# salemmohammed/Distributed-TensorFlow-Guide

Hardware: AMD Instinct MI355X
Metric: images/sec (whole node) ResNet-50 sync DP at 1/2/4/8 MI355X; scaling efficiency (higher is better)
Workload: dtype bf16; 1 GPU; model=ResNet-50, global_batch=1024, per_gpu_batch=1024, image_size=224, optimizer=momentum-sgd (fused), parallelism=dp1, allreduce=rccl bf16, 8 MB buckets, overlapped, step_launch=eager

## Files before the change

### csrc/bindings/ops.cc

```cpp
#include <torch/extension.h>
#include <c10/core/DeviceGuard.h>
#include <c10/hip/HIPStream.h>

#include "dtg/kernels.h"

namespace {

using at::Tensor;
using dtg::bf16_t;

hipStream_t cur_stream() { return c10::hip::getCurrentHIPStream().stream(); }

at::Tensor zeros_f32(long long n, const at::Tensor& like) {
  c10::DeviceGuard dg(like.device());
  at::Tensor t = at::empty({n}, like.options().dtype(at::kFloat));
  dtg::fill_zero(t.data_ptr(), n * 4, cur_stream());
  return t;
}

#define CHECK_CUDA(x) TORCH_CHECK((x).is_cuda(), #x " must be a GPU tensor")
#define CHECK_CONTIG(x) TORCH_CHECK((x).is_contiguous(), #x " must be contiguous")
#define CHECK_DT(x, dt) TORCH_CHECK((x).scalar_type() == (dt), #x " must be " #dt)
#define CHECK_IN(x) \
  CHECK_CUDA(x);    \
// ... 987 lines not shown
  CHECK_IN(x);
  CHECK_DT(x, at::kBFloat16);
  TORCH_CHECK(x.dim() == 2, "x must be [M, C]");
  const long long M = x.size(0);
  const int C = (int)x.size(1);
  TORCH_CHECK(C % 8 == 0, "C must be a multiple of 8");
  check_partials({&part}, C);
  check_per_channel({&gamma, &beta, &rmean, &rvar}, C);
  const bool has_res = res.has_value() && res->defined();
  if (has_res) {
    CHECK_IN(*res);
    CHECK_DT(*res, at::kBFloat16);
    TORCH_CHECK(res->sizes() == x.sizes(), "residual shape mismatch");
  }
  c10::DeviceGuard dg(x.device());
  auto y = at::empty_like(x);
  auto fopt = x.options().dtype(at::kFloat);
  auto smean = at::empty({C}, fopt), sinv = at::empty({C}, fopt), ws = at::empty({2LL * C}, fopt);
  dtg::bn_fwd_from_part(cbfp(x), has_res ? cbfp(*res) : nullptr, bfp(y), gamma.data_ptr<float>(),
                        beta.data_ptr<float>(), rmean.data_ptr<float>(), rvar.data_ptr<float>(),
                        smean.data_ptr<float>(), sinv.data_ptr<float>(), part.data_ptr<float>(), ws.data_ptr<float>(),
                        M, C, (float)momentum, (float)eps, relu, cur_stream(), bits_ptr(bits, M, C));
  return {y, smean, sinv};
}

std::tuple<Tensor, Tensor, Tensor, Tensor, Tensor> bn_fwd2_part(Tensor x, Tensor part, Tensor gamma, Tensor beta,
                                                                Tensor rmean, Tensor rvar, Tensor r, Tensor part2,
                                                                Tensor gamma2, Tensor beta2, Tensor rmean2,
                                                                Tensor rvar2, double momentum, double eps,
                                                                c10::optional<Tensor> bits) {
  CHECK_IN(x);
  CHECK_IN(r);
  CHECK_DT(x, at::kBFloat16);
  CHECK_DT(r, at::kBFloat16);
  TORCH_CHECK(x.dim() == 2 && r.sizes() == x.sizes(), "x/r must be [M, C]");
  const long long M = x.size(0);
  const int C = (int)x.size(1);
  TORCH_CHECK(C % 8 == 0, "C must be a multiple of 8");
  check_partials({&part, &part2}, C);
  check_per_channel({&gamma, &beta, &rmean, &rvar, &gamma2, &beta2, &rmean2, &rvar2}, C);
  c10::DeviceGuard dg(x.device());
  auto y = at::empty_like(x);
  auto fopt = x.options().dtype(at::kFloat);
  auto m1 = at::empty({C}, fopt), i1 = at::empty({C}, fopt), m2 = at::empty({C}, fopt), i2 = at::empty({C}, fopt);
  auto ws = at::empty({4LL * C}, fopt);
  dtg::bn_fwd2_from_part(cbfp(x), cbfp(r), bfp(y), part.data_ptr<float>(), part2.data_ptr<float>(),
// ... 256 lines not shown
  m.def("bn_dx_wgrad_ok", [](int64_t M, int64_t C, int64_t CI) { return dtg::bn_dx_wgrad_ok(M, (int)C, (int)CI); });
  m.def("bn_dx_dgrad_ok", [](int64_t M, int64_t C, int64_t CI) { return dtg::bn_dx_dgrad_ok(M, (int)C, (int)CI); });
  m.def("bn_dx_dgrad_full_ok",
        [](int64_t M, int64_t C, int64_t CI) { return dtg::bn_dx_dgrad_full_ok(M, (int)C, (int)CI); });
  m.def("bn_dx_wgrad_slabs",
        [](int64_t C, int64_t CI, int64_t w2, bool dg) { return dtg::bn_dx_wgrad_slabs((int)C, (int)CI, (int)w2, dg); },
        pybind11::arg("C"), pybind11::arg("CI"), pybind11::arg("w2") = 0, pybind11::arg("dg") = false);
  m.def("conv_fwd_bn", &conv_fwd_bn, pybind11::arg("x"), pybind11::arg("w"), pybind11::arg("stride"),
        pybind11::arg("pad"), pybind11::arg("pooled") = false);
  m.def("conv_dgrad_bn", &conv_dgrad_bn, pybind11::arg("dy"), pybind11::arg("w"), pybind11::arg("H"),
        pybind11::arg("W"), pybind11::arg("stride"), pybind11::arg("pad"), pybind11::arg("x"), pybind11::arg("mean"),
        pybind11::arg("invstd"), pybind11::arg("gamma"), pybind11::arg("beta"), pybind11::arg("pooled") = false,
        pybind11::arg("bits") = pybind11::none());
  m.def("bn_fwd2_part", &bn_fwd2_part, pybind11::arg("x"), pybind11::arg("part"), pybind11::arg("gamma"),
        pybind11::arg("beta"), pybind11::arg("rmean"), pybind11::arg("rvar"), pybind11::arg("r"), pybind11::arg("part2"),
        pybind11::arg("gamma2"), pybind11::arg("beta2"), pybind11::arg("rmean2"), pybind11::arg("rvar2"),
        pybind11::arg("momentum"), pybind11::arg("eps"), pybind11::arg("bits") = pybind11::none());
  m.def("conv_fwd_c8", &conv_fwd_c8, pybind11::arg("x"), pybind11::arg("w"), pybind11::arg("R"), pybind11::arg("S"),
        pybind11::arg("stride"), pybind11::arg("pad"), pybind11::arg("with_stats") = false,
        pybind11::arg("stride_w") = 0);
  m.def("bn_fwd_part", &bn_fwd_part, pybind11::arg("x"), pybind11::arg("part"), pybind11::arg("res"),
        pybind11::arg("gamma"), pybind11::arg("beta"), pybind11::arg("rmean"), pybind11::arg("rvar"),
        pybind11::arg("momentum"), pybind11::arg("eps"), pybind11::arg("relu"), pybind11::arg("bits") = pybind11::none());
  m.def("bn_bwd_part", &bn_bwd_part, pybind11::arg("dp"), pybind11::arg("x"), pybind11::arg("part"),
        pybind11::arg("gamma"), pybind11::arg("smean"), pybind11::arg("sinv"), pybind11::arg("want_dres"),
        pybind11::arg("dgamma_acc") = pybind11::none(), pybind11::arg("dbeta_acc") = pybind11::none(),
        pybind11::arg("wact") = pybind11::none(), pybind11::arg("wgrad") = pybind11::none(),
        pybind11::arg("dgw") = pybind11::none(), pybind11::arg("dgy") = pybind11::none(),
        pybind11::arg("dgmean") = pybind11::none(), pybind11::arg("dginv") = pybind11::none(),
        pybind11::arg("dgbits") = pybind11::none(), pybind11::arg("dgpart") = pybind11::none(),
        pybind11::arg("dgfull") = false);
  m.doc() = "dtg gfx950 HIP kernels";
  {
    namespace py = pybind11;
    m.def("sgd_apply", &sgd_apply, py::arg("w"), py::arg("mirror"), py::arg("g"), py::arg("hyper"), py::arg("wd"),
          py::arg("gscale"), py::arg("zero_grad"), py::arg("clip") = py::none());
    m.def("momentum_apply", &momentum_apply, py::arg("w"), py::arg("mirror"), py::arg("g"), py::arg("mom"),
          py::arg("hyper"), py::arg("mu"), py::arg("wd"), py::arg("nesterov"), py::arg("gscale"), py::arg("zero_grad"),
          py::arg("clip") = py::none());
    m.def("adagrad_apply", &adagrad_apply, py::arg("w"), py::arg("mirror"), py::arg("g"), py::arg("acc"),
          py::arg("hyper"), py::arg("eps"), py::arg("gscale"), py::arg("zero_grad"), py::arg("clip") = py::none());
    m.def("adam_apply", &adam_apply, py::arg("w"), py::arg("mirror"), py::arg("g"), py::arg("m"), py::arg("v"),
          py::arg("hyper"), py::arg("b1"), py::arg("b2"), py::arg("eps"), py::arg("wd"), py::arg("gscale"),
          py::arg("zero_grad"), py::arg("clip") = py::none());
  }
  m.attr("LW_CHUNK") = (int)dtg::kLwChunk;
// ... 28 lines not shown
      sbytes = scratch->numel() * scratch->element_size();
      dev_t = &*scratch;
    }
    if (bucket.has_value() && bucket->defined()) {
      CHECK_IN(*bucket);
      TORCH_CHECK(bucket->scalar_type() == at::kFloat || bucket->scalar_type() == at::kBFloat16, "bucket fp32/bf16");
      n = bucket->numel();
      bf = bucket->scalar_type() == at::kBFloat16;
      dev_t = &*bucket;
    }
    TORCH_CHECK(!(mode & 2) || sbytes > 0, "traffic mode needs scratch");
    TORCH_CHECK(!(mode & 4) || n > 0 || !(bucket.has_value() && bucket->defined()), "data mode needs the bucket");
    c10::optional<c10::DeviceGuard> dg;
    if (dev_t) dg.emplace(dev_t->device());
    return dtg::comm_emu(seconds, (int)wgs, (int)mode, sbytes ? scratch->data_ptr() : nullptr, sbytes, base,
                         traffic_bytes, n ? bucket->data_ptr() : nullptr, n, bf, (float)factor, cur_stream());
  }, pybind11::arg("seconds"), pybind11::arg("wgs") = 32, pybind11::arg("mode") = 0,
        pybind11::arg("scratch") = pybind11::none(), pybind11::arg("base") = 0, pybind11::arg("traffic_bytes") = 0,
        pybind11::arg("bucket") = pybind11::none(), pybind11::arg("factor") = 1.0);
  m.def("stem_stream_set", [](int64_t on) { dtg::stem_stream_set((int)on); });
  m.def("gemm_expand_k256_set", [](int64_t on) { dtg::gemm_expand_k256_set((int)on); });
  m.def("stem_pool_rows_set", [](int64_t on) { dtg::stem_pool_rows_set((int)on); });
  m.def("gemm_expand_s2_set", [](int64_t on) { dtg::gemm_expand_s2_set((int)on); });
  m.def("conv_halo_fwd_set", [](int64_t on) { dtg::conv3x3_halo_fwd_set((int)on); });
  m.def("conv_halo_dgrad_set", [](int64_t on) { dtg::conv3x3_halo_dgrad_set((int)on); });
  m.def("conv_halo_wgrad_set", [](int64_t on) { dtg::conv3x3_halo_wgrad_set((int)on); });
  m.def("conv_lin_wgrad_set", [](int64_t on) { dtg::conv3x3_lin_wgrad_set((int)on); });
  m.def("hyper_tick", [](Tensor hyper) {
    check_hyper(hyper);
    c10::DeviceGuard dg(hyper.device());
    dtg::hyper_tick(hyper.data_ptr<float>(), cur_stream());
  });
  m.def("stem_pack_weights", [](Tensor w) {
    CHECK_CUDA(w);
    CHECK_DT(w, at::kBFloat16);
    TORCH_CHECK(w.dim() == 4 && w.is_contiguous(at::MemoryFormat::ChannelsLast) && w.size(1) <= 4,
                "w: channels_last [K, C<=4, R, S]");
    const int K = w.size(0), C = w.size(1), R = w.size(2), S = w.size(3), S2 = (S + 1) / 2;
    const int KP = (R * S2 * 8 + 63) / 64 * 64;
    c10::DeviceGuard dg(w.device());
    auto wp = at::empty({K, KP}, w.options().memory_format(at::MemoryFormat::Contiguous));
    dtg::stem_pack_weights(cbfp(w), bfp(wp), K, C, R, S, S2, KP, cur_stream());
    return wp;
  });
  m.def("stem_dw_add", [](Tensor src, Tensor grad, bool pair) {
    CHECK_IN(src);
// ... 63 lines not shown
```

### csrc/include/dtg/kernels.h

```cpp
#pragma once
#include <hip/hip_runtime.h>
#include <stdint.h>

namespace dtg {
typedef unsigned short bf16_t;

void sgd_apply(float* w, bf16_t* mirror, void* grad, int grad_bf16, long long n, const float* hyper, float wd,
               float gscale, int zero_grad, hipStream_t st, const float* clip = nullptr);
void momentum_apply(float* w, bf16_t* mirror, void* grad, int grad_bf16, float* mom, long long n,
                    const float* hyper, float mu, float wd, int nesterov, float gscale, int zero_grad,
                    hipStream_t st, const float* clip = nullptr);
void adagrad_apply(float* w, bf16_t* mirror, void* grad, int grad_bf16, float* acc, long long n,
                   const float* hyper, float eps, float gscale, int zero_grad, hipStream_t st,
                   const float* clip = nullptr);
void adam_apply(float* w, bf16_t* mirror, void* grad, int grad_bf16, float* m, float* v, long long n,
                const float* hyper, float b1, float b2, float eps, float wd, float gscale, int zero_grad,
                hipStream_t st, const float* clip = nullptr);
void axpby(float* acc, const void* g, int g_bf16, long long n, float alpha, float beta, hipStream_t st);
void f32_to_bf16(const float* x, bf16_t* y, long long n, hipStream_t st);
void hyper_tick(float* hyper, hipStream_t st);
struct GradSrcs {
  const void* p[8] = {nullptr, nullptr, nullptr, nullptr, nullptr, nullptr, nullptr, nullptr};
};
void sgd_sum_apply(float* w, bf16_t* mirror, const float* acc, const GradSrcs& src, int k, int src_bf16, long long n,
// ... 235 lines not shown
int conv_supported(int C, int K, int R, int S, int stride, int pad, int which);
int conv3x3_halo_bn_ok(int C, int K, int H, int W);
bool conv3x3_halo_bn_fwd(const bf16_t* x, const bf16_t* w, bf16_t* y, int N, int H, int W, float* part, hipStream_t st);
void conv3x3_halo_fwd_set(int on);
bool conv3x3_halo_bn_dgrad(const bf16_t* dy, const bf16_t* w, bf16_t* dp, int N, int H, int W, const BnEpi& bn,
                           hipStream_t st);
void conv3x3_halo_dgrad_set(int on);
int conv3x3_halo_wgrad_split(int N, int H, int W, int C, int K, int R, int S, int stride, int pad, int stride_w);
void conv3x3_halo_wgrad(const bf16_t* dy, const bf16_t* x, float* ws, int grid, int N, int H, hipStream_t st);
void conv3x3_halo_wgrad_set(int on);
int conv3x3_lin_wgrad_split(int N, int H, int W, int C, int K, int R, int S, int stride, int pad, int stride_w);
void conv3x3_lin_wgrad(const bf16_t* dy, const bf16_t* x, float* ws, int split, int N, int H, int W, int C, int K,
                       hipStream_t st);
void conv3x3_lin_wgrad_set(int on);
void conv_fwd(const bf16_t* x, const bf16_t* w, bf16_t* y, int N, int H, int W, int C, int K, int R, int S,
              int stride, int pad, hipStream_t st, const BnEpi& bn = BnEpi());
int conv_dgrad(const bf16_t* dy, const bf16_t* w, bf16_t* dx, int N, int H, int W, int C, int K, int R, int S,
               int stride, int pad, float beta, hipStream_t st, const BnEpi& bn = BnEpi(),
               const bf16_t* wT = nullptr, int zero_rest = 1);
void stem_stream_set(int on);
void stem_pool_rows_set(int on);
void gemm_expand_k256_set(int on);
void gemm_expand_s2_set(int on);
bool conv1x1_s2_expand_bn(const bf16_t* x, int Nb, int H, int W, int Cin, const bf16_t* w, bf16_t* y, int Kout,
                          float* part, hipStream_t st);
void conv_fwd_c8(const bf16_t* x, const bf16_t* w, bf16_t* y, int N, int H, int W, int K, int R, int S, int stride,
                 int pad, hipStream_t st, const BnEpi& bn = BnEpi(), int stride_w = 0);
void conv_set_stages(int which, int stages);
int conv_wgrad_split(int N, int H, int W, int C, int K, int R, int S, int stride, int pad, int stride_w = 0,
                     int target_wgs = 0);
void conv_wgrad(const bf16_t* dy, const bf16_t* x, void* dw, int dw_bf16, float beta, float* ws, int split, int N,
                int H, int W, int C, int K, int R, int S, int stride, int pad, hipStream_t st, int stride_w = 0,
                int sched = 0);

}
```

### csrc/kernels/batchnorm.hip

```cpp
#include <stdlib.h>
#include "dtg/common.h"
#include "dtg/kernels.h"
#include "dtg/bn_finalize.cuh"

namespace dtg {

long long bn_workspace_floats(long long M, int C) {
  BnGeom g = bn_geom(M, C);
  return (long long)g.nchunk * 2 * C + 4LL * C;
}

template <int TPR>
__global__ void __launch_bounds__(kBlk) bn_stats_kernel(const bf16_t* __restrict__ x, long long M, int C,
                                                        long long rpc, float* __restrict__ part) {
  constexpr int RPP = kBlk / TPR, CW = TPR * 8;
  __shared__ float sh[2][RPP][CW + 4];
  const int tx = threadIdx.x % TPR, ty = threadIdx.x / TPR;
  const int c0 = blockIdx.y * CW + tx * 8;
  const long long m0 = (long long)blockIdx.x * rpc;
  const long long m1 = m0 + rpc < M ? m0 + rpc : M;
  float s[8] = {0, 0, 0, 0, 0, 0, 0, 0}, q[8] = {0, 0, 0, 0, 0, 0, 0, 0};
  if (c0 < C) {
    long long m = m0 + ty;
    for (; m + RPP < m1; m += 2 * RPP) {
// ... 266 lines not shown
      if (relu) { bn_apply_kernel<T, false, true, RU><<<ga, kBlk, 0, st>>>(x, res, y, coef, M, C, rpa, bits); DTG_LAUNCH_CHECK(); }
      else { bn_apply_kernel<T, false, false, RU><<<ga, kBlk, 0, st>>>(x, res, y, coef, M, C, rpa, bits); DTG_LAUNCH_CHECK(); }
    }
  }));
}

void bn_fwd_train(const bf16_t* x, const bf16_t* res, bf16_t* y, const float* gamma, const float* beta,
                  float* rmean, float* rvar, float* smean, float* sinv, float* ws, long long M, int C,
                  float momentum, float eps, int relu, hipStream_t st) {
  const BnGeom g = bn_geom(M, C);
  float* part = ws;
  float* coef = ws + (long long)g.nchunk * 2 * C;
  dim3 grid(g.nchunk, g.gy);
  DTG_TPR_SWITCH(g.tpr, bn_stats_kernel<T><<<grid, kBlk, 0, st>>>(x, M, C, g.rows_per_chunk, part)); DTG_LAUNCH_CHECK();
  bn_finalize_kernel<16><<<(C + 63) / 64, 1024, 0, st>>>(part, g.nchunk, M, C, 0, gamma, beta, rmean, rvar, smean, sinv,
                                                    momentum, eps, coef, nullptr, nullptr); DTG_LAUNCH_CHECK();
  bn_apply_launch(g, x, res, y, coef, M, C, relu, st);
}

void bn_fwd_from_part(const bf16_t* x, const bf16_t* res, bf16_t* y, const float* gamma, const float* beta,
                      float* rmean, float* rvar, float* smean, float* sinv, const float* part, float* ws, long long M,
                      int C, float momentum, float eps, int relu, hipStream_t st, uint8_t* bits) {
  const BnGeom g = bn_geom(M, C);
  bn_finalize_kernel<16><<<(C + 63) / 64, 1024, 0, st>>>(part, kBnStatSlots, M, C, 0, gamma, beta, rmean, rvar, smean,
                                                    sinv, momentum, eps, ws, nullptr, nullptr, 1); DTG_LAUNCH_CHECK();
  bn_apply_launch(g, x, res, y, ws, M, C, relu, st, bits);
}

__global__ void bn_infer_coef_kernel(const float* gamma, const float* beta, const float* rmean, const float* rvar,
                                     float eps, int C, float* coef) {
  const int c = blockIdx.x * blockDim.x + threadIdx.x;
  if (c >= C) return;
  const float inv = rsqrtf(rvar[c] + eps);
  const float sc = (gamma ? gamma[c] : 1.f) * inv;
  coef[c] = sc;
  coef[C + c] = (beta ? beta[c] : 0.f) - rmean[c] * sc;
}

void bn_fwd_infer(const bf16_t* x, const bf16_t* res, bf16_t* y, const float* gamma, const float* beta,
                  const float* rmean, const float* rvar, float* ws, long long M, int C, float eps, int relu,
                  hipStream_t st) {
  const BnGeom g = bn_geom(M, C);
  float* coef = ws;
  bn_infer_coef_kernel<<<(C + 255) / 256, 256, 0, st>>>(gamma, beta, rmean, rvar, eps, C, coef); DTG_LAUNCH_CHECK();
  dim3 grid(g.nchunk, g.gy);
  const long long rpa = elementwise_rpc(g, M);
  dim3 ga((unsigned)((M + rpa - 1) / rpa), g.gy);
  DTG_TPR_SWITCH(g.tpr, {
    if (res) {
// ... 151 lines not shown
```

### csrc/kernels/gemm_expand.hip

```cpp
#include "dtg/common.h"
#include "dtg/kernels.h"
#include "dtg/mfma_gemm.cuh"

namespace dtg {

namespace {
using namespace gemm;

constexpr int kXR = 64;
constexpr int kXS = 3;

struct ExpandGather {
  int H, W;
  FastDiv fPQ, fQ;
};

template <int K, bool NT, int MINB, bool S2 = false>
__global__ void __launch_bounds__(256, MINB > 0 ? MINB : 1) gemm_expand_bn_kernel(const bf16_t* __restrict__ A, long long lda,
                                                             const bf16_t* __restrict__ W, long long ldw,
                                                             bf16_t* __restrict__ C, long long ldc,
                                                             float* __restrict__ part, int N, int nslice, int tiles,
                                                             ExpandGather gth) {
  constexpr int KS = K / 32;
  constexpr int KH = K / 64;
  constexpr int BLK = kXR * K * 2;
  constexpr int D = KH * 2;
  constexpr int T = 8;
  __shared__ __attribute__((aligned(16))) char smem_raw[kXS * BLK];
  lds_char* smem = (lds_char*)smem_raw;
  const int tid = threadIdx.x, lane = tid & 63;
  const int wave = __builtin_amdgcn_readfirstlane(tid >> 6);
  const int G = gridDim.x;
  const int base = xcd_remap(blockIdx.x, G);
  const int my = base < tiles ? (tiles - base + G - 1) / G : 0;
  if (my == 0) return;
  const int slice = base % nslice;
  const int col0 = slice * 256 + wave * 64;
  const int q = lane & 15, g = lane >> 4;

  v8bf wf[4][KS];
#pragma unroll
  for (int j = 0; j < 4; ++j)
#pragma unroll
    for (int ks = 0; ks < KS; ++ks) {
      const int n = col0 + 32 * (j >> 1) + 8 * (q >> 2) + 4 * (j & 1) + (q & 3);
      wf[j][ks] = *reinterpret_cast<const v8bf*>(W + (long long)n * ldw + ks * 32 + 8 * g);
    }

  const int rb0 = base / nslice, gs = G / nslice;
  auto stage = [&](int it) {
// ... 3 lines not shown
    for (int i = 0; i < 2; ++i) {
      const int r0 = (wave * 2 + i) * 8, r = r0 + (lane >> 3);
      const int c = (lane & 7) ^ (r & 7);
      long long arow = (long long)rb * kXR + r;
      if constexpr (S2) {
        uint32_t n, pq, pp, qq;
        gth.fPQ.divmod((uint32_t)arow, n, pq);
        gth.fQ.divmod(pq, pp, qq);
        arow = ((long long)n * gth.H + 2 * (int)pp) * gth.W + 2 * (int)qq;
      }
      const char* src = (const char*)(A + arow * lda + c * 8);
#pragma unroll
      for (int h = 0; h < KH; ++h)
        __builtin_amdgcn_global_load_lds((const void*)(src + h * 128), (lds_void*)(dst + h * kXR * 128 + r0 * 128), 16,
                                         0, 0);
    }
  };

  float s[16], sq[16];
#pragma unroll
  for (int c = 0; c < 16; ++c) s[c] = sq[c] = 0.f;
  const f32x4 zero4 = {0.f, 0.f, 0.f, 0.f};

  stage(0);
  stage(1);
  for (int it = 0; it < my; ++it) {
    if (it == 0) asm volatile("s_waitcnt vmcnt(%0)" ::"n"(D) : "memory");
    else if (it == 1) asm volatile("s_waitcnt vmcnt(%0)" ::"n"(D + T) : "memory");
    else asm volatile("s_waitcnt vmcnt(%0)" ::"n"(2 * T + D) : "memory");
    __builtin_amdgcn_s_barrier();
    stage(it + 2);
    const lds_char* ta = smem + (it % kXS) * BLK;
    const long long row0 = (long long)(rb0 + it * gs) * kXR;
#pragma unroll
    for (int i = 0; i < 4; ++i) {
      v8bf af[KS];
#pragma unroll
      for (int ks = 0; ks < KS; ++ks) af[ks] = frag_kc(ta + (ks >> 1) * kXR * 128, 16 * i, ks & 1, lane);
      f32x4 acc[4];
#pragma unroll
      for (int j = 0; j < 4; ++j) acc[j] = __builtin_amdgcn_mfma_f32_16x16x32_bf16(wf[j][0], af[0], zero4, 0, 0, 0);
#pragma unroll
      for (int ks = 1; ks < KS; ++ks)
#pragma unroll
        for (int j = 0; j < 4; ++j)
          acc[j] = __builtin_amdgcn_mfma_f32_16x16x32_bf16(wf[j][ks], af[ks], acc[j], 0, 0, 0);
      u32x4v w0, w1;
      w0.x = pack_bf2(acc[0][0], acc[0][1]);
      w0.y = pack_bf2(acc[0][2], acc[0][3]);
      w0.z = pack_bf2(acc[1][0], acc[1][1]);
      w0.w = pack_bf2(acc[1][2], acc[1][3]);
      w1.x = pack_bf2(acc[2][0], acc[2][1]);
      w1.y = pack_bf2(acc[2][2], acc[2][3]);
      w1.z = pack_bf2(acc[3][0], acc[3][1]);
      w1.w = pack_bf2(acc[3][2], acc[3][3]);
      const uint32_t wd[8] = {w0.x, w0.y, w0.z, w0.w, w1.x, w1.y, w1.z, w1.w};
#pragma unroll
      for (int c = 0; c < 8; ++c) {
        const float lo = __uint_as_float(wd[c] << 16), hi = __uint_as_float(wd[c] & 0xffff0000u);
        s[2 * c] += lo;
        s[2 * c + 1] += hi;
        sq[2 * c] = fmaf(lo, lo, sq[2 * c]);
        sq[2 * c + 1] = fmaf(hi, hi, sq[2 * c + 1]);
      }
      bf16_t* dst = C + (row0 + 16 * i + q) * ldc + col0 + 8 * g;
      if constexpr (NT) {
        __builtin_nontemporal_store(w0, reinterpret_cast<u32x4v*>(dst));
        __builtin_nontemporal_store(w1, reinterpret_cast<u32x4v*>(dst + 32));
      } else {
        *reinterpret_cast<u32x4v*>(dst) = w0;
        *reinterpret_cast<u32x4v*>(dst + 32) = w1;
      }
    }
  }
  asm volatile("s_waitcnt vmcnt(0)" ::: "memory");

#pragma unroll
  for (int c = 0; c < 16; ++c) {
#pragma unroll
    for (int o = 1; o < 16; o <<= 1) {
      s[c] += __shfl_xor(s[c], o, 64);
      sq[c] += __shfl_xor(sq[c], o, 64);
    }
  }
  if (q == 0) {
    float* p = part + (long long)(blockIdx.x % kBnStatSlots) * 2 * N + col0 + 8 * g;
#pragma unroll
    for (int c = 0; c < 16; ++c) {
      const int off = c < 8 ? c : 24 + c;
      atomicAdd(p + off, s[c]);
      atomicAdd(p + N + off, sq[c]);
    }
  }
}

template <int K, bool NT, int MINB, bool S2 = false>
int expand_grid(int nslice) {
  static int per_cu = -1, cus = 0;
  if (per_cu < 0) {
    int dev = 0;
    DTG_HIP_CHECK(hipGetDevice(&dev));
    DTG_HIP_CHECK(hipDeviceGetAttribute(&cus, hipDeviceAttributeMultiprocessorCount, dev));
    DTG_HIP_CHECK(hipOccupancyMaxActiveBlocksPerMultiprocessor(&per_cu, gemm_expand_bn_kernel<K, NT, MINB, S2>, 256, 0));
    if (per_cu < 1) per_cu = 1;
  }
  int G = cus * per_cu;
  const int mult = nslice > 8 ? nslice : 8;
  G -= G % mult;
  return G > 0 ? G : mult;
}

struct StemStreamGeom {
  int Hp, Wp2, P, Q;
  FastDiv fPQ, fQ;
};

__global__ void __launch_bounds__(256, 2) stem_stream_bn_kernel(const bf16_t* __restrict__ x8,
                                                                 const bf16_t* __restrict__ W,
                                                                 bf16_t* __restrict__ C, float* __restrict__ part,
                                                                 StemStreamGeom sg, int nblocks) {
  constexpr int K = 256, KS = K / 32, KH = K / 64, N = 64;
  constexpr int BLK = kXR * K * 2;
  constexpr int D = KH * 2;
  constexpr int T = 2;
  constexpr int TAPS = 28;
  constexpr int RING = 2;
// ... 96 lines not shown
    for (int c = 0; c < 16; ++c) {
      const int off = c < 8 ? c : 24 + c;
      atomicAdd(pp + off, s[c]);
      atomicAdd(pp + N + off, sq[c]);
    }
  }
}

}

static int g_expand_k256 = 1;
void gemm_expand_k256_set(int on) { g_expand_k256 = on; }

bool gemm_expand_bn(const bf16_t* A, long long lda, const bf16_t* W, long long ldw, bf16_t* C, long long ldc, int M,
                    int N, int K, float* part, hipStream_t st, int variant) {
  if ((K != 64 && K != 128 && !(K == 256 && g_expand_k256)) || N % 256 || M % kXR || (lda & 7) || (ldw & 7) ||
      (ldc & 7))
    return false;
  if ((long long)M * N < (1LL << 24)) return false;
  const int nslice = N / 256;
  if (nslice & (nslice - 1)) return false;
  const int tiles = (M / kXR) * nslice;
  auto launch = [&](auto kern, int G) {
    hipLaunchKernelGGL(kern, dim3(G), dim3(256), 0, st, A, lda, W, ldw, C, ldc, part, N, nslice, tiles, ExpandGather());
  };
  if (K == 64) {
    if (variant == 1) launch(gemm_expand_bn_kernel<64, true, 0>, expand_grid<64, true, 0>(nslice));
    else if (variant == 2) launch(gemm_expand_bn_kernel<64, false, 3>, expand_grid<64, false, 3>(nslice));
    else launch(gemm_expand_bn_kernel<64, false, 0>, expand_grid<64, false, 0>(nslice));
  } else if (K == 256) {
    launch(gemm_expand_bn_kernel<256, false, 0>, expand_grid<256, false, 0>(nslice));
  } else {
    if (variant == 1) launch(gemm_expand_bn_kernel<128, true, 0>, expand_grid<128, true, 0>(nslice));
    else if (variant == 2) launch(gemm_expand_bn_kernel<128, false, 2>, expand_grid<128, false, 2>(nslice));
    else launch(gemm_expand_bn_kernel<128, false, 0>, expand_grid<128, false, 0>(nslice));
  }
  DTG_LAUNCH_CHECK();
  return true;
}

static int g_expand_s2 = 1;
void gemm_expand_s2_set(int on) { g_expand_s2 = on; }

bool conv1x1_s2_expand_bn(const bf16_t* x, int Nb, int H, int W, int Cin, const bf16_t* w, bf16_t* y, int Kout,
                          float* part, hipStream_t st) {
  if (!g_expand_s2 || Cin != 256 || Kout % 256 || (H & 1) || (W & 1)) return false;
  const int P = H / 2, Q = W / 2;
  const long long M = (long long)Nb * P * Q;
  if (M % kXR || M >= (1LL << 31) || (long long)Nb * H * W * Cin >= (1LL << 40)) return false;
  if (M * Kout < (1LL << 24)) return false;
  const int nslice = Kout / 256;
  if (nslice & (nslice - 1)) return false;
  ExpandGather gth;
  gth.H = H;
  gth.W = W;
  gth.fPQ = FastDiv((uint32_t)(P * Q));
  gth.fQ = FastDiv((uint32_t)Q);
  const int tiles = (int)(M / kXR) * nslice;
  hipLaunchKernelGGL((gemm_expand_bn_kernel<256, false, 0, true>), dim3(expand_grid<256, false, 0, true>(nslice)),
                     dim3(256), 0, st, x, (long long)Cin, w, (long long)Cin, y, (long long)Kout, part, Kout, nslice, tiles,
                     gth);
  DTG_LAUNCH_CHECK();
  return true;
}

static int g_stem_stream = 1;
void stem_stream_set(int on) { g_stem_stream = on; }

bool stem_conv_stream_bn(const bf16_t* x8, const bf16_t* w8, bf16_t* y, int N, int Hp, int Wp2, int P, int Q,
                         float* part, hipStream_t st) {
  if (!g_stem_stream) return false;
  const long long M = (long long)N * P * Q;
  if (M % kXR || M / kXR > (1LL << 30) || (long long)N * Hp * Wp2 * 8 >= (1LL << 31)) return false;
  if (2 * (P - 1) + 7 > Hp || (Q - 1) + 4 > Wp2) return false;
  StemStreamGeom sg;
  sg.Hp = Hp;
  sg.Wp2 = Wp2;
  sg.P = P;
  sg.Q = Q;
  sg.fPQ = FastDiv((uint32_t)(P * Q));
  sg.fQ = FastDiv((uint32_t)Q);
  static int G = 0;
  if (G == 0) {
    int dev = 0, cus = 0, per_cu = 0;
    DTG_HIP_CHECK(hipGetDevice(&dev));
    DTG_HIP_CHECK(hipDeviceGetAttribute(&cus, hipDeviceAttributeMultiprocessorCount, dev));
// ... 12 lines not shown
```

### distributed-tensorflow-guide_amd/models/resnet_fused.py

```python
import os

import torch
import torch.nn.functional as F

from ..ops import conv as conv_ops
from ..ops._native import lib
from ..ops.gemm import gemm
from ..parallel import grad_sink, overlap


def _rows(t):
    n, c, h, w = t.shape
    if not t.is_contiguous(memory_format=torch.channels_last):
        t = t.contiguous(memory_format=torch.channels_last)
    return t.permute(0, 2, 3, 1).reshape(n * h * w, c)


def _mat(w):
    return w.reshape(w.shape[0], w.shape[1]) if w.is_contiguous() else w.as_strided((w.shape[0], w.shape[1]),
                                                                                     (w.shape[1], 1))


def _krsc(w):
    return w.permute(0, 2, 3, 1)


_FUSE = True
_LINK = True
_SUB2 = True
_DXW = True
_DXW2 = True
_DXD = True
_DXD2 = True
_DXD_S2 = True
_dxd_calls = 0


class _Bn3Link:
    __slots__ = ("y3", "m3", "i3", "gamma", "beta", "bits", "yd", "md", "idd", "part", "part2", "dp")

    def __init__(self, y3, m3, i3, gamma, beta, bits, yd=None, md=None, idd=None):
        self.y3, self.m3, self.i3, self.gamma, self.beta = y3, m3, i3, gamma, beta
        self.bits = bits
        self.yd, self.md, self.idd = yd, md, idd
        self.part = self.part2 = self.dp = None


def _gacc(p):
    if grad_sink.enabled(p):
        return p.grad, True
    return torch.zeros_like(p, dtype=torch.float32 if p.dim() <= 1 else p.dtype), False


_BITS = True


_WSPLIT_WGS = int(os.environ.get("DTG_RESNET_WSPLIT_WGS", "256"))
_CWSPLIT_WGS = int(os.environ.get("DTG_RESNET_CWSPLIT_WGS", "256"))
# ... 19 lines not shown

class _BottleneckFn(torch.autograd.Function):
    @staticmethod
    def forward(ctx, x, blk, link_in, holder, *params):
        L = lib()
        n, c, h, w = x.shape
        st = blk.c2.conv.stride
        width = blk.c1.conv.weight.shape[0]
        cout = blk.c3.conv.weight.shape[0]
        x2 = _rows(x)
        p_, q_ = (h + 2 - 3) // st + 1, (w + 2 - 3) // st + 1
        b1, b2, b3 = blk.c1.bn, blk.c2.bn, blk.c3.bn
        w1, w2, w3 = blk.c1.conv.weight, blk.c2.conv.weight, blk.c3.conv.weight
        if _FUSE:
            y1, p1 = L.gemm_bn(x2, _mat(w1), 1, pooled=True)
            bits1 = _relu_bits(y1)
            a1, m1, i1 = L.bn_fwd_part(y1, p1, None, b1.weight, b1.bias, b1.running_mean, b1.running_var,
                                       b1.momentum, b1.eps, True, bits=bits1)
            y2, p2 = L.conv_fwd_bn(a1.view(n, h, w, width), _krsc(w2), st, 1, pooled=True)
            y2 = y2.view(-1, width)
            bits2 = _relu_bits(y2)
            a2, m2, i2 = L.bn_fwd_part(y2, p2, None, b2.weight, b2.bias, b2.running_mean, b2.running_var,
                                       b2.momentum, b2.eps, True, bits=bits2)
            y3, p3 = L.gemm_bn(a2, _mat(w3), 1, pooled=True)
            ctx.bits12 = (bits1, bits2)
        else:
            y1 = gemm(x2, True, _mat(w1), True)
            a1, m1, i1 = L.bn_fwd_train(y1, None, b1.weight, b1.bias, b1.running_mean, b1.running_var, b1.momentum,
                                        b1.eps, True)
            y2 = L.conv_fwd(a1.view(n, h, w, width), _krsc(w2), st, 1).view(-1, width)
            a2, m2, i2 = L.bn_fwd_train(y2, None, b2.weight, b2.bias, b2.running_mean, b2.running_var, b2.momentum,
                                        b2.eps, True)
            y3 = gemm(a2, True, _mat(w3), True)
        yd = md = idd = None
        if blk.down is not None:
            bd, wd = blk.down.bn, blk.down.conv.weight
            if _FUSE:
                if st == 1:
                    yd, pd = L.gemm_bn(x2, _mat(wd), 1, pooled=True)
                else:
                    yd, pd = L.conv_fwd_bn(x2.view(n, h, w, c), _krsc(wd), st, 0, pooled=True)
                    yd = yd.view(-1, cout)
                idn = None
            else:
                if st == 1:
                    yd = gemm(x2, True, _mat(wd), True)
                else:
                    yd = L.conv_fwd(x2.view(n, h, w, c), _krsc(wd), st, 0).view(-1, cout)
                idn, md, idd = L.bn_fwd_train(yd, None, bd.weight, bd.bias, bd.running_mean, bd.running_var,
                                              bd.momentum, bd.eps, False)
        else:
            idn = x2
        bits = None
        if _FUSE and _LINK:
            bits = torch.empty(y3.shape[0], cout // 8, device=y3.device, dtype=torch.uint8)
        if _FUSE and blk.down is not None:
            assert bd.momentum == b3.momentum and bd.eps == b3.eps
            out, m3, i3, md, idd = L.bn_fwd2_part(y3, p3, b3.weight, b3.bias, b3.running_mean, b3.running_var, yd, pd,
                                                  bd.weight, bd.bias, bd.running_mean, bd.running_var, b3.momentum,
                                                  b3.eps, bits=bits)
        elif _FUSE:
            out, m3, i3 = L.bn_fwd_part(y3, p3, idn, b3.weight, b3.bias, b3.running_mean, b3.running_var,
                                        b3.momentum, b3.eps, True, bits=bits)
        else:
            out, m3, i3 = L.bn_fwd_train(y3, idn, b3.weight, b3.bias, b3.running_mean, b3.running_var, b3.momentum,
                                         b3.eps, True)
        ctx.blk = blk
        ctx.link_in = link_in if (_FUSE and _LINK) else None
        ctx.link_out = _Bn3Link(y3, m3, i3, b3.weight, b3.bias, bits, yd, md, idd) if (_FUSE and _LINK) else None
        holder.append(ctx.link_out)
        ctx.geom = (n, c, h, w, st, width, cout, p_, q_)
        ctx.save_for_backward(x2, y1, a1, m1, i1, y2, a2, m2, i2, y3, out, m3, i3,
                              *((yd, md, idd) if yd is not None else ()))
        return out.view(n, p_, q_, cout).permute(0, 3, 1, 2)

    @staticmethod
    def backward(ctx, dout):
        L = lib()
        blk = ctx.blk
# ... 253 lines not shown
```

Measured before the change: 16870 images/sec.

## Recompute expand GEMM in a fused BN-apply pass instead of storing then rereading

For non-downsample bottleneck blocks, the final 1x1 expand conv now runs twice. The first pass computes only the BN partial statistics without storing its output. After the statistics are finalized, a second pass recomputes the GEMM and fuses BN scale/shift, the residual add, ReLU, the output store and the ReLU bitmask store. This replaces a full write and reread of the pre-BN activation with extra GEMM compute, since the GEMM has small K. The apply pass still writes y3 for backward, so it trades one activation read for a second GEMM and more register pressure.

Result: no change. 16970 images/sec, median of 6 (+0.6%).

```diff
diff --git a/csrc/bindings/ops.cc b/csrc/bindings/ops.cc
--- a/csrc/bindings/ops.cc
+++ b/csrc/bindings/ops.cc
@@ -1033,6 +1033,52 @@
                         smean.data_ptr<float>(), sinv.data_ptr<float>(), part.data_ptr<float>(), ws.data_ptr<float>(),
                         M, C, (float)momentum, (float)eps, relu, cur_stream(), bits_ptr(bits, M, C));
   return {y, smean, sinv};
+}
+
+static void check_expand_operands(const Tensor& A, const Tensor& W, const char* what) {
+  CHECK_IN(A);
+  CHECK_DT(A, at::kBFloat16);
+  CHECK_CUDA(W);
+  CHECK_DT(W, at::kBFloat16);
+  TORCH_CHECK(A.dim() == 2 && W.dim() == 2 && W.stride(1) == 1 && W.size(1) == A.size(1), what,
+              ": A [M, K], W [N, K] with contiguous rows");
+  TORCH_CHECK(W.stride(0) % 8 == 0 && ((uintptr_t)A.data_ptr() % 16) == 0 && ((uintptr_t)W.data_ptr() % 16) == 0, what,
+              ": 16-byte aligned rows");
+  TORCH_CHECK(dtg::gemm_expand_apply_ok(A.size(0), (int)W.size(0), (int)A.size(1)), what,
+              ": shape not served (K in {64, 128, 256}, N % 256 == 0 with N / 256 a power of two, M % 64 == 0)");
+}
+
+Tensor gemm_expand_stats(Tensor A, Tensor W) {
+  check_expand_operands(A, W, "gemm_expand_stats");
+  const int M = (int)A.size(0), K = (int)A.size(1), N = (int)W.size(0);
+  c10::DeviceGuard dg(A.device());
+  auto part = bn_part(A, N, true);
+  dtg::gemm_expand_stats(cbfp(A), A.stride(0), cbfp(W), W.stride(0), M, N, K, part.data_ptr<float>(), cur_stream());
+  return part;
+}
+
+std::tuple<Tensor, Tensor, Tensor, Tensor> bn_fwd_part_gemm(Tensor A, Tensor W, Tensor part, Tensor res, Tensor gamma,
+                                                            Tensor beta, Tensor rmean, Tensor rvar, double momentum,
+                                                            double eps, Tensor bits) {
+  check_expand_operands(A, W, "bn_fwd_part_gemm");
+  const int M = (int)A.size(0), K = (int)A.size(1), N = (int)W.size(0);
+  check_partials({&part}, N);
+  check_per_channel({&gamma, &beta, &rmean, &rvar}, N);
+  CHECK_IN(res);
+  CHECK_DT(res, at::kBFloat16);
+  TORCH_CHECK(res.dim() == 2 && res.size(0) == M && res.size(1) == N, "residual shape mismatch");
+  uint8_t* bp = bits_ptr(bits, M, N);
+  TORCH_CHECK(bp != nullptr, "bn_fwd_part_gemm needs the bits tensor");
+  c10::DeviceGuard dg(A.device());
+  auto y = at::empty({M, N}, A.options()), out = at::empty({M, N}, A.options());
+  auto fopt = A.options().dtype(at::kFloat);
+  auto smean = at::empty({N}, fopt), sinv = at::empty({N}, fopt), coef = at::empty({2LL * N}, fopt);
+  dtg::bn_finalize_part(gamma.data_ptr<float>(), beta.data_ptr<float>(), rmean.data_ptr<float>(), rvar.data_ptr<float>(),
+                        smean.data_ptr<float>(), sinv.data_ptr<float>(), part.data_ptr<float>(), coef.data_ptr<float>(),
+                        M, N, (float)momentum, (float)eps, cur_stream());
+  dtg::gemm_expand_apply(cbfp(A), A.stride(0), cbfp(W), W.stride(0), bfp(y), cbfp(res), bfp(out), coef.data_ptr<float>(),
+                         bp, M, N, K, cur_stream());
+  return {y, out, smean, sinv};
 }
 
 std::tuple<Tensor, Tensor, Tensor, Tensor, Tensor> bn_fwd2_part(Tensor x, Tensor part, Tensor gamma, Tensor beta,
@@ -1335,6 +1381,16 @@
   m.def("bn_fwd_part", &bn_fwd_part, pybind11::arg("x"), pybind11::arg("part"), pybind11::arg("res"),
         pybind11::arg("gamma"), pybind11::arg("beta"), pybind11::arg("rmean"), pybind11::arg("rvar"),
         pybind11::arg("momentum"), pybind11::arg("eps"), pybind11::arg("relu"), pybind11::arg("bits") = pybind11::none());
+  m.def("gemm_expand_stats", &gemm_expand_stats, pybind11::arg("A"), pybind11::arg("W"));
+  m.def("bn_fwd_part_gemm", &bn_fwd_part_gemm, pybind11::arg("A"), pybind11::arg("W"), pybind11::arg("part"),
+        pybind11::arg("res"), pybind11::arg("gamma"), pybind11::arg("beta"), pybind11::arg("rmean"), pybind11::arg("rvar"),
+        pybind11::arg("momentum"), pybind11::arg("eps"), pybind11::arg("bits"));
+  m.def("gemm_expand_apply_ok",
+        [](int64_t M, int64_t N, int64_t K) { return dtg::gemm_expand_apply_ok(M, (int)N, (int)K); });
+  m.def("gemm_expand_form_grid", [](int64_t K, int64_t nslice, int64_t form) {
+    TORCH_CHECK((K == 64 || K == 128 || K == 256) && nslice >= 1 && (form == 1 || form == 2), "K, nslice or form");
+    return dtg::gemm_expand_form_grid((int)K, (int)nslice, (int)form);
+  });
   m.def("bn_bwd_part", &bn_bwd_part, pybind11::arg("dp"), pybind11::arg("x"), pybind11::arg("part"),
         pybind11::arg("gamma"), pybind11::arg("smean"), pybind11::arg("sinv"), pybind11::arg("want_dres"),
         pybind11::arg("dgamma_acc") = pybind11::none(), pybind11::arg("dbeta_acc") = pybind11::none(),
@@ -1409,6 +1465,7 @@
   m.def("gemm_expand_k256_set", [](int64_t on) { dtg::gemm_expand_k256_set((int)on); });
   m.def("stem_pool_rows_set", [](int64_t on) { dtg::stem_pool_rows_set((int)on); });
   m.def("gemm_expand_s2_set", [](int64_t on) { dtg::gemm_expand_s2_set((int)on); });
+  m.def("gemm_expand_apply_nt_set", [](int64_t on) { dtg::gemm_expand_apply_nt_set((int)on); });
   m.def("conv_halo_fwd_set", [](int64_t on) { dtg::conv3x3_halo_fwd_set((int)on); });
   m.def("conv_halo_dgrad_set", [](int64_t on) { dtg::conv3x3_halo_dgrad_set((int)on); });
   m.def("conv_halo_wgrad_set", [](int64_t on) { dtg::conv3x3_halo_wgrad_set((int)on); });
diff --git a/csrc/include/dtg/kernels.h b/csrc/include/dtg/kernels.h
--- a/csrc/include/dtg/kernels.h
+++ b/csrc/include/dtg/kernels.h
@@ -281,6 +281,15 @@
 void stem_pool_rows_set(int on);
 void gemm_expand_k256_set(int on);
 void gemm_expand_s2_set(int on);
+bool gemm_expand_apply_ok(long long M, int N, int K);
+void gemm_expand_apply_nt_set(int on);
+int gemm_expand_form_grid(int K, int nslice, int form);
+void gemm_expand_stats(const bf16_t* A, long long lda, const bf16_t* W, long long ldw, int M, int N, int K, float* part,
+                       hipStream_t st);
+void gemm_expand_apply(const bf16_t* A, long long lda, const bf16_t* W, long long ldw, bf16_t* y, const bf16_t* res,
+                       bf16_t* out, const float* coef, uint8_t* bits, int M, int N, int K, hipStream_t st);
+void bn_finalize_part(const float* gamma, const float* beta, float* rmean, float* rvar, float* smean, float* sinv,
+                      const float* part, float* coef, long long M, int C, float momentum, float eps, hipStream_t st);
 bool conv1x1_s2_expand_bn(const bf16_t* x, int Nb, int H, int W, int Cin, const bf16_t* w, bf16_t* y, int Kout,
                           float* part, hipStream_t st);
 void conv_fwd_c8(const bf16_t* x, const bf16_t* w, bf16_t* y, int N, int H, int W, int K, int R, int S, int stride,
diff --git a/csrc/kernels/batchnorm.hip b/csrc/kernels/batchnorm.hip
--- a/csrc/kernels/batchnorm.hip
+++ b/csrc/kernels/batchnorm.hip
@@ -312,9 +312,14 @@
                       float* rmean, float* rvar, float* smean, float* sinv, const float* part, float* ws, long long M,
                       int C, float momentum, float eps, int relu, hipStream_t st, uint8_t* bits) {
   const BnGeom g = bn_geom(M, C);
+  bn_finalize_part(gamma, beta, rmean, rvar, smean, sinv, part, ws, M, C, momentum, eps, st);
+  bn_apply_launch(g, x, res, y, ws, M, C, relu, st, bits);
+}
+
+void bn_finalize_part(const float* gamma, const float* beta, float* rmean, float* rvar, float* smean, float* sinv,
+                      const float* part, float* coef, long long M, int C, float momentum, float eps, hipStream_t st) {
   bn_finalize_kernel<16><<<(C + 63) / 64, 1024, 0, st>>>(part, kBnStatSlots, M, C, 0, gamma, beta, rmean, rvar, smean,
-                                                    sinv, momentum, eps, ws, nullptr, nullptr, 1); DTG_LAUNCH_CHECK();
-  bn_apply_launch(g, x, res, y, ws, M, C, relu, st, bits);
+                                                    sinv, momentum, eps, coef, nullptr, nullptr, 1); DTG_LAUNCH_CHECK();
 }
 
 __global__ void bn_infer_coef_kernel(const float* gamma, const float* beta, const float* rmean, const float* rvar,
diff --git a/csrc/kernels/gemm_expand.hip b/csrc/kernels/gemm_expand.hip
--- a/csrc/kernels/gemm_expand.hip
+++ b/csrc/kernels/gemm_expand.hip
@@ -15,17 +15,34 @@
   FastDiv fPQ, fQ;
 };
 
-template <int K, bool NT, int MINB, bool S2 = false>
+struct ExpandApply {
+  const bf16_t* res;
+  bf16_t* out;
+  const float* coef;
+  uint8_t* bits;
+};
+
+__device__ __forceinline__ uint32_t relu_bits8(const float (&v)[8]) {
+  uint32_t b = 0;
+#pragma unroll
+  for (int k = 0; k < 8; ++k) b |= (v[k] > 0.f ? 1u : 0u) << k;
+  return b;
+}
+
+enum { kFormStore = 0, kFormStats = 1, kFormApply = 2 };
+
+template <int K, bool NT, int MINB, bool S2 = false, int FORM = kFormStore>
 __global__ void __launch_bounds__(256, MINB > 0 ? MINB : 1) gemm_expand_bn_kernel(const bf16_t* __restrict__ A, long long lda,
                                                              const bf16_t* __restrict__ W, long long ldw,
                                                              bf16_t* __restrict__ C, long long ldc,
                                                              float* __restrict__ part, int N, int nslice, int tiles,
-                                                             ExpandGather gth) {
+                                                             ExpandGather gth, ExpandApply ap) {
   constexpr int KS = K / 32;
   constexpr int KH = K / 64;
   constexpr int BLK = kXR * K * 2;
   constexpr int D = KH * 2;
-  constexpr int T = 8;
+  constexpr int T = FORM == kFormStore ? 8 : FORM == kFormStats ? 0 : 4 * 5 + 8;
+  static_assert((FORM == kFormApply ? T + 8 : 2 * T) + D <= 63, "the 6-bit vmcnt");
   __shared__ __attribute__((aligned(16))) char smem_raw[kXS * BLK];
   lds_char* smem = (lds_char*)smem_raw;
   const int tid = threadIdx.x, lane = tid & 63;
@@ -75,14 +92,45 @@
   for (int c = 0; c < 16; ++c) s[c] = sq[c] = 0.f;
   const f32x4 zero4 = {0.f, 0.f, 0.f, 0.f};
 
+  float sc[16], sf[16];
+  u32x4v rr[4][2];
+  if constexpr (FORM == kFormApply) {
+#pragma unroll
+    for (int h = 0; h < 2; ++h) {
+      float t0[8], t1[8];
+      load8_f32(ap.coef + col0 + 32 * h + 8 * g, t0);
+      load8_f32(ap.coef + N + col0 + 32 * h + 8 * g, t1);
+#pragma unroll
+      for (int c = 0; c < 8; ++c) sc[8 * h + c] = t0[c], sf[8 * h + c] = t1[c];
+    }
+#pragma unroll
+    for (int j = 0; j < 4; ++j)
+#pragma unroll
+      for (int ks = 0; ks < KS; ++ks) asm volatile("" : "+v"(wf[j][ks]));
+#pragma unroll
+    for (int c = 0; c < 16; ++c) asm volatile("" : "+v"(sc[c]), "+v"(sf[c]));
+  }
+
+  auto res_load = [&](int it, int i) {
+    const int rb = rb0 + (it < my ? it : my - 1) * gs;
+    const bf16_t* src = ap.res + ((long long)rb * kXR + 16 * i + q) * N + col0 + 8 * g;
+    rr[i][0] = *reinterpret_cast<const u32x4v*>(src);
+    rr[i][1] = *reinterpret_cast<const u32x4v*>(src + 32);
+  };
   stage(0);
   stage(1);
+  if constexpr (FORM == kFormApply) {
+    asm volatile("" ::: "memory");
+#pragma unroll
+    for (int i = 0; i < 4; ++i) res_load(0, i);
+  }
   for (int it = 0; it < my; ++it) {
+    constexpr int W1 = FORM == kFormApply ? D + T + 8 : D + T, W2 = FORM == kFormApply ? D + T + 8 : 2 * T + D;
     if (it == 0) asm volatile("s_waitcnt vmcnt(%0)" ::"n"(D) : "memory");
-    else if (it == 1) asm volatile("s_waitcnt vmcnt(%0)" ::"n"(D + T) : "memory");
-    else asm volatile("s_waitcnt vmcnt(%0)" ::"n"(2 * T + D) : "memory");
+    else if (it == 1) asm volatile("s_waitcnt vmcnt(%0)" ::"n"(W1) : "memory");
+    else asm volatile("s_waitcnt vmcnt(%0)" ::"n"(W2) : "memory");
     __builtin_amdgcn_s_barrier();
-    stage(it + 2);
+    if constexpr (FORM != kFormApply) stage(it + 2);
     const lds_char* ta = smem + (it % kXS) * BLK;
     const long long row0 = (long long)(rb0 + it * gs) * kXR;
 #pragma unroll
@@ -107,26 +155,72 @@
       w1.y = pack_bf2(acc[2][2], acc[2][3]);
       w1.z = pack_bf2(acc[3][0], acc[3][1]);
       w1.w = pack_bf2(acc[3][2], acc[3][3]);
-      const uint32_t wd[8] = {w0.x, w0.y, w0.z, w0.w, w1.x, w1.y, w1.z, w1.w};
-#pragma unroll
-      for (int c = 0; c < 8; ++c) {
-        const float lo = __uint_as_float(wd[c] << 16), hi = __uint_as_float(wd[c] & 0xffff0000u);
-        s[2 * c] += lo;
-        s[2 * c + 1] += hi;
-        sq[2 * c] = fmaf(lo, lo, sq[2 * c]);
-        sq[2 * c + 1] = fmaf(hi, hi, sq[2 * c + 1]);
+      if constexpr (FORM != kFormApply) {
+        const uint32_t wd[8] = {w0.x, w0.y, w0.z, w0.w, w1.x, w1.y, w1.z, w1.w};
+#pragma unroll
+        for (int c = 0; c < 8; ++c) {
+          const float lo = __uint_as_float(wd[c] << 16), hi = __uint_as_float(wd[c] & 0xffff0000u);
+          s[2 * c] += lo;
+          s[2 * c + 1] += hi;
+          sq[2 * c] = fmaf(lo, lo, sq[2 * c]);
+          sq[2 * c + 1] = fmaf(hi, hi, sq[2 * c + 1]);
+        }
       }
-      bf16_t* dst = C + (row0 + 16 * i + q) * ldc + col0 + 8 * g;
-      if constexpr (NT) {
-        __builtin_nontemporal_store(w0, reinterpret_cast<u32x4v*>(dst));
-        __builtin_nontemporal_store(w1, reinterpret_cast<u32x4v*>(dst + 32));
-      } else {
-        *reinterpret_cast<u32x4v*>(dst) = w0;
-        *reinterpret_cast<u32x4v*>(dst + 32) = w1;
+      if constexpr (FORM != kFormStats) {
+        bf16_t* dst = C + (row0 + 16 * i + q) * ldc + col0 + 8 * g;
+        if constexpr (NT) {
+          __builtin_nontemporal_store(w0, reinterpret_cast<u32x4v*>(dst));
+          __builtin_nontemporal_store(w1, reinterpret_cast<u32x4v*>(dst + 32));
+        } else {
+          *reinterpret_cast<u32x4v*>(dst) = w0;
+          *reinterpret_cast<u32x4v*>(dst + 32) = w1;
+        }
       }
+      if constexpr (FORM == kFormApply) {
+        float o[2][8];
+        u32x4v ow[2];
+#pragma unroll
+        for (int h = 0; h < 2; ++h) {
+          float r[8];
+          unpack8_bf16(h ? w1 : w0, o[h]);
+          unpack8_bf16(rr[i][h], r);
+#pragma unroll
+          for (int k = 0; k < 8; ++k) {
+            float v = o[h][k] * sc[8 * h + k] + sf[8 * h + k];
+            v += r[k];
+            v = fmaxf(v, 0.f);
+            o[h][k] = v;
+          }
+          ow[h].x = pack_bf2(o[h][0], o[h][1]);
+          ow[h].y = pack_bf2(o[h][2], o[h][3]);
+          ow[h].z = pack_bf2(o[h][4], o[h][5]);
+          ow[h].w = pack_bf2(o[h][6], o[h][7]);
+        }
+        const long long orow = row0 + 16 * i + q;
+        bf16_t* od = ap.out + orow * N + col0 + 8 * g;
+        *reinterpret_cast<u32x4v*>(od) = ow[0];
+        *reinterpret_cast<u32x4v*>(od + 32) = ow[1];
+        uint32_t bw = (relu_bits8(o[0]) | (relu_bits8(o[1]) << 16)) << (8 * (g & 1));
+        bw |= __shfl_xor(bw, 16, 64);
+        const uint32_t bo = __shfl_xor(bw, 32, 64);
+        {
+          const uint32_t lo = g < 2 ? bw : bo, hi = g < 2 ? bo : bw;
+          const uint32_t x = (lo & 0xffffu) | (hi << 16), y = (lo >> 16) | (hi & 0xffff0000u);
+          const uint16_t b2 = (uint16_t)((g < 2 ? x : y) >> (16 * (g & 1)));
+          *reinterpret_cast<uint16_t*>(ap.bits + orow * (N >> 3) + (col0 >> 3) + 2 * g) = b2;
+        }
+      }
+    }
+    if constexpr (FORM == kFormApply) {
+      asm volatile("" ::: "memory");
+      stage(it + 2);
+      asm volatile("" ::: "memory");
+#pragma unroll
+      for (int i = 0; i < 4; ++i) res_load(it + 1, i);
     }
   }
   asm volatile("s_waitcnt vmcnt(0)" ::: "memory");
+  if constexpr (FORM == kFormApply) return;
 
 #pragma unroll
   for (int c = 0; c < 16; ++c) {
@@ -147,14 +241,15 @@
   }
 }
 
-template <int K, bool NT, int MINB, bool S2 = false>
+template <int K, bool NT, int MINB, bool S2 = false, int FORM = kFormStore>
 int expand_grid(int nslice) {
   static int per_cu = -1, cus = 0;
   if (per_cu < 0) {
     int dev = 0;
     DTG_HIP_CHECK(hipGetDevice(&dev));
     DTG_HIP_CHECK(hipDeviceGetAttribute(&cus, hipDeviceAttributeMultiprocessorCount, dev));
-    DTG_HIP_CHECK(hipOccupancyMaxActiveBlocksPerMultiprocessor(&per_cu, gemm_expand_bn_kernel<K, NT, MINB, S2>, 256, 0));
+    DTG_HIP_CHECK(hipOccupancyMaxActiveBlocksPerMultiprocessor(&per_cu, gemm_expand_bn_kernel<K, NT, MINB, S2, FORM>, 256,
+                                                               0));
     if (per_cu < 1) per_cu = 1;
   }
   int G = cus * per_cu;
@@ -297,7 +392,8 @@
   if (nslice & (nslice - 1)) return false;
   const int tiles = (M / kXR) * nslice;
   auto launch = [&](auto kern, int G) {
-    hipLaunchKernelGGL(kern, dim3(G), dim3(256), 0, st, A, lda, W, ldw, C, ldc, part, N, nslice, tiles, ExpandGather());
+    hipLaunchKernelGGL(kern, dim3(G), dim3(256), 0, st, A, lda, W, ldw, C, ldc, part, N, nslice, tiles, ExpandGather(),
+                       ExpandApply());
   };
   if (K == 64) {
     if (variant == 1) launch(gemm_expand_bn_kernel<64, true, 0>, expand_grid<64, true, 0>(nslice));
@@ -334,9 +430,60 @@
   const int tiles = (int)(M / kXR) * nslice;
   hipLaunchKernelGGL((gemm_expand_bn_kernel<256, false, 0, true>), dim3(expand_grid<256, false, 0, true>(nslice)),
                      dim3(256), 0, st, x, (long long)Cin, w, (long long)Cin, y, (long long)Kout, part, Kout, nslice, tiles,
-                     gth);
+                     gth, ExpandApply());
   DTG_LAUNCH_CHECK();
   return true;
+}
+
+bool gemm_expand_apply_ok(long long M, int N, int K) {
+  if (K != 64 && K != 128 && K != 256) return false;
+  if (M <= 0 || N <= 0 || N % 256 || M % kXR || M * (long long)N >= (1LL << 40) || M / kXR >= (1LL << 24)) return false;
+  const int nslice = N / 256;
+  return (nslice & (nslice - 1)) == 0;
+}
+
+template <int FORM, bool NT = false, class F>
+static void expand_form_dispatch(int K, int nslice, F&& f) {
+  if (K == 64) f(gemm_expand_bn_kernel<64, NT, 0, false, FORM>, expand_grid<64, NT, 0, false, FORM>(nslice));
+  else if (K == 128) f(gemm_expand_bn_kernel<128, NT, 0, false, FORM>, expand_grid<128, NT, 0, false, FORM>(nslice));
+  else f(gemm_expand_bn_kernel<256, NT, 0, false, FORM>, expand_grid<256, NT, 0, false, FORM>(nslice));
+}
+
+static int g_expand_apply_nt = 0;
+void gemm_expand_apply_nt_set(int on) { g_expand_apply_nt = on; }
+
+int gemm_expand_form_grid(int K, int nslice, int form) {
+  int G = 0;
+  if (form == kFormStats) expand_form_dispatch<kFormStats>(K, nslice, [&](auto, int g) { G = g; });
+  else expand_form_dispatch<kFormApply>(K, nslice, [&](auto, int g) { G = g; });
+  return G;
+}
+
+void gemm_expand_stats(const bf16_t* A, long long lda, const bf16_t* W, long long ldw, int M, int N, int K, float* part,
+                       hipStream_t st) {
+  const int nslice = N / 256, tiles = (M / kXR) * nslice;
+  expand_form_dispatch<kFormStats>(K, nslice, [&](auto kern, int G) {
+    hipLaunchKernelGGL(kern, dim3(G), dim3(256), 0, st, A, lda, W, ldw, (bf16_t*)nullptr, (long long)N, part, N, nslice,
+                       tiles, ExpandGather(), ExpandApply());
+  });
+  DTG_LAUNCH_CHECK();
+}
+
+void gemm_expand_apply(const bf16_t* A, long long lda, const bf16_t* W, long long ldw, bf16_t* y, const bf16_t* res,
+                       bf16_t* out, const float* coef, uint8_t* bits, int M, int N, int K, hipStream_t st) {
+  const int nslice = N / 256, tiles = (M / kXR) * nslice;
+  ExpandApply ap;
+  ap.res = res;
+  ap.out = out;
+  ap.coef = coef;
+  ap.bits = bits;
+  auto launch = [&](auto kern, int G) {
+    hipLaunchKernelGGL(kern, dim3(G), dim3(256), 0, st, A, lda, W, ldw, y, (long long)N, (float*)nullptr, N, nslice,
+                       tiles, ExpandGather(), ap);
+  };
+  if (g_expand_apply_nt) expand_form_dispatch<kFormApply, true>(K, nslice, launch);
+  else expand_form_dispatch<kFormApply>(K, nslice, launch);
+  DTG_LAUNCH_CHECK();
 }
 
 static int g_stem_stream = 1;
diff --git a/distributed-tensorflow-guide_amd/models/resnet_fused.py b/distributed-tensorflow-guide_amd/models/resnet_fused.py
--- a/distributed-tensorflow-guide_amd/models/resnet_fused.py
+++ b/distributed-tensorflow-guide_amd/models/resnet_fused.py
@@ -34,6 +34,9 @@
 _DXD2 = True
 _DXD_S2 = True
 _dxd_calls = 0
+_C3A = 7
+_C3A_MIN = 1 << 24
+_c3a_calls = 0
 
 
 class _Bn3Link:
@@ -99,7 +102,12 @@
             bits2 = _relu_bits(y2)
             a2, m2, i2 = L.bn_fwd_part(y2, p2, None, b2.weight, b2.bias, b2.running_mean, b2.running_var,
                                        b2.momentum, b2.eps, True, bits=bits2)
-            y3, p3 = L.gemm_bn(a2, _mat(w3), 1, pooled=True)
+            c3a = (_LINK and blk.down is None and (_C3A & (width // 64)) and width in (64, 128, 256)
+                   and a2.shape[0] * cout >= _C3A_MIN and L.gemm_expand_apply_ok(a2.shape[0], cout, width))
+            if c3a:
+                y3, p3 = None, L.gemm_expand_stats(a2, _mat(w3))
+            else:
+                y3, p3 = L.gemm_bn(a2, _mat(w3), 1, pooled=True)
             ctx.bits12 = (bits1, bits2)
         else:
             y1 = gemm(x2, True, _mat(w1), True)
@@ -109,6 +117,7 @@
             a2, m2, i2 = L.bn_fwd_train(y2, None, b2.weight, b2.bias, b2.running_mean, b2.running_var, b2.momentum,
                                         b2.eps, True)
             y3 = gemm(a2, True, _mat(w3), True)
+            c3a = False
         yd = md = idd = None
         if blk.down is not None:
             bd, wd = blk.down.bn, blk.down.conv.weight
@@ -130,8 +139,13 @@
             idn = x2
         bits = None
         if _FUSE and _LINK:
-            bits = torch.empty(y3.shape[0], cout // 8, device=y3.device, dtype=torch.uint8)
-        if _FUSE and blk.down is not None:
+            bits = torch.empty(a2.shape[0], cout // 8, device=a2.device, dtype=torch.uint8)
+        if _FUSE and c3a:
+            global _c3a_calls
+            _c3a_calls += 1
+            y3, out, m3, i3 = L.bn_fwd_part_gemm(a2, _mat(w3), p3, idn, b3.weight, b3.bias, b3.running_mean,
+                                                 b3.running_var, b3.momentum, b3.eps, bits)
+        elif _FUSE and blk.down is not None:
             assert bd.momentum == b3.momentum and bd.eps == b3.eps
             out, m3, i3, md, idd = L.bn_fwd2_part(y3, p3, b3.weight, b3.bias, b3.running_mean, b3.running_var, yd, pd,
                                                   bd.weight, bd.bias, bd.running_mean, bd.running_var, b3.momentum,
```
